# florianbaud/retrieval-augmented-mds

Hardware: AMD Instinct MI355X
Metric: MIPS queries/sec (exact top-5, bf16 index) (higher is better)
Workload: dtype bf16

## Files before the change

retrieval-augmented-mds_amd/csrc/scan_kernel_v4.hpp:

```cpp
#pragma once
#include <hip/hip_runtime.h>
#include <stdint.h>

#include "scan_kernel.hpp"
#include "scan_kernel_v3.hpp"

namespace mips {

typedef float f32x4 __attribute__((ext_vector_type(4)));

__device__ __forceinline__ unsigned lane_id_here() {
    unsigned ln = 0;
#if defined(__HIP_DEVICE_COMPILE__)
    asm volatile("v_mbcnt_lo_u32_b32 %0, -1, 0\n\tv_mbcnt_hi_u32_b32 %0, -1, %0" : "=v"(ln));
#endif
    return ln;
}

template <int KL, int KS32, int AD, int = 0, bool NT_DOCS = false, int PUB = 1>
__global__ __launch_bounds__(512, 2) void scan_kernel_v4(ScanArgs p) {
    extern __shared__ __attribute__((aligned(16))) unsigned char smem[];
    constexpr int WAVES = 8;
    constexpr int TN = WAVES * 32;
    constexpr int STAGES = 3;
    constexpr int STAGE_BYTES = V3_DB * KS32 * 64;
    constexpr int PIECES = STAGE_BYTES / 1024;
    constexpr int PPW = PIECES / WAVES;
    static_assert(PIECES % WAVES == 0, "every wave must issue the same number of DMA pieces");
    static_assert(KL <= 8, "8 class words vouch for 8 documents");
    static_assert(PUB >= 1 && PUB <= KL, "a sub-list publishes one of its entries");
    constexpr int STEPS = 2 * KS32;
    constexpr bool ONE_PASS = KL == 6 && KS32 == 24 && !NT_DOCS && PUB == 1;
    constexpr int KLI = ONE_PASS ? 4 : KL;
    static_assert(PUB <= KLI, "a sub-list publishes one of the entries it keeps");

    const int tid = threadIdx.x;
    const int lane = tid & 63;
    const int wave = __builtin_amdgcn_readfirstlane(tid >> 6);
    const int c = lane & 15;
    const int g = lane >> 4;

    const int xcd = blockIdx.x & 7;
    const int j = blockIdx.x >> 3;
    const int qt = (xcd % p.qgroups) + p.qgroups * (j % p.qt_per_group);
    const int split = (xcd / p.qgroups) * p.splits_per_group + j / p.qt_per_group;
    if (qt >= p.nqt) return;
    if (p.spin_limit < 0 && tid == 0) *p.err = 1u;
    const bool idle_wave = (qt * TN + wave * 32) >= p.nq;

    const int b0 = split * p.tiles_per_split;
    int b1 = b0 + p.tiles_per_split;
    if (b1 > p.ntiles) b1 = p.ntiles;
    const int nb = b1 > b0 ? b1 - b0 : 0;

    bf16x8 bq[2][KS32];
#pragma unroll
    for (int n = 0; n < 2; ++n) {
        const uint16_t* qrow = p.qbuf + ((int64_t)qt * TN + wave * 32 + n * 16 + c) * p.ld + 8 * g;
#pragma unroll
        for (int s = 0; s < KS32; ++s) bq[n][s] = *reinterpret_cast<const bf16x8*>(qrow + 32 * s);
#if defined(__HIP_DEVICE_COMPILE__)
#pragma unroll
        for (int s = 0; s < KS32; ++s) asm volatile("" : "+v"(bq[n][s]));
#endif
    }

    float ls[2][KLI];
    int li[2][KLI];
    float thr[2];
#pragma unroll
    for (int n = 0; n < 2; ++n) {
        thr[n] = -INFINITY;
#pragma unroll
        for (int i = 0; i < KLI; ++i) {
            ls[n][i] = -INFINITY;
            li[n][i] = IDX_NONE;
        }
    }

    constexpr unsigned THR_AREA = STAGES * STAGE_BYTES;
    constexpr unsigned THR_WAVE = 1024u;
    constexpr unsigned DUMP_AREA = THR_AREA + WAVES * THR_WAVE;
    static_assert(THR_AREA % 1024 == 0, "the wave areas are recovered from thr_addr by masking");
    auto thr_addr_of = [&](unsigned ln) { return THR_AREA + wave * THR_WAVE + ln * 16u; };
    *reinterpret_cast<uint4*>(smem + thr_addr_of(lane)) = make_uint4(0u, 0u, 0u, 0u);
    const __amdgpu_buffer_rsrc_t thr_rsrc = __builtin_amdgcn_make_buffer_rsrc(
        (void*)(reinterpret_cast<unsigned char*>(p.gthr) + (int64_t)qt * (WAVES * THR_WAVE) - (int64_t)THR_AREA), 0,
        (int)(THR_AREA + WAVES * THR_WAVE), 0x00020000);
    auto refresh_thresholds = [&](bool real) {
        lds_void* dst = (lds_void*)(smem + (real ? THR_AREA + wave * THR_WAVE : DUMP_AREA));
        const unsigned thr_addr = thr_addr_of(lane_id_here());
        __builtin_amdgcn_raw_ptr_buffer_load_lds(thr_rsrc, dst, 16, real ? thr_addr : (thr_addr | 0x40000000u), 0, 0, 16);
    };

    const unsigned char* docs_b = reinterpret_cast<const unsigned char*>(p.docs);
    const int64_t row_bytes = (int64_t)p.ld * 2;
    unsigned lane_off_kept = 0u;
    if constexpr (ONE_PASS) {
        lane_off_kept = ((unsigned)lane >> 3) * (unsigned)row_bytes + ((((unsigned)lane & 7u) ^ (((unsigned)lane >> 4) & 7u)) << 4);
#if defined(__HIP_DEVICE_COMPILE__)
        asm volatile("" : "+v"(lane_off_kept));
#endif
    }
    auto issue_piece = [&](const unsigned char* blk_base, int stage, int i) {
        const __amdgpu_buffer_rsrc_t rsrc =
            __builtin_amdgcn_make_buffer_rsrc((void*)blk_base, 0, (int)(V3_DB * row_bytes), 0x00020000);
        const int pc = wave + WAVES * i;
        const int slab = pc >> 2, rg = pc & 3;
        unsigned lane_off0 = lane_off_kept;
        if constexpr (!ONE_PASS) {
            const unsigned ln = __builtin_amdgcn_mbcnt_hi(~0u, __builtin_amdgcn_mbcnt_lo(~0u, 0u));
            lane_off0 = (ln >> 3) * (unsigned)row_bytes + (((ln & 7u) ^ ((ln >> 4) & 7u)) << 4);
        }
        __builtin_amdgcn_raw_ptr_buffer_load_lds(rsrc, (lds_void*)(smem + stage * STAGE_BYTES + pc * 1024), 16,
                                                 (rg & 1) ? (lane_off0 ^ 64u) : lane_off0,
                                                 rg * 8 * (int)row_bytes + slab * 128, 0, NT_DOCS ? 2 : 0);
    };
    auto issue = [&](const unsigned char* blk_base, int stage) {
#pragma unroll
        for (int i = 0; i < PPW; ++i) issue_piece(blk_base, stage, i);
    };

    auto rd0_of = [&](unsigned ln) {
        const unsigned cc = ln & 15u, gg = ln >> 4;
        return (int)(cc * 128u + ((gg ^ ((cc >> 1) & 7u)) << 4));
    };

    const unsigned cnt_lds = (unsigned)(size_t)(lds_void*)(smem + DUMP_AREA + 1024);
    unsigned arrivals_needed = 0;
    constexpr int PER_BLOCK = PPW + 1;
    auto arrive = [&]() {
        asm volatile("s_waitcnt vmcnt(%0)" ::"n"((STAGES - 2) * PER_BLOCK) : "memory");
#if defined(__HIP_DEVICE_COMPILE__)
        if (lane == 0) asm volatile("ds_add_u32 %0, %1" ::"v"(cnt_lds), "v"(1u) : "memory");
#endif
    };
    auto wait_all = [&]() {
        arrivals_needed += WAVES;
        for (int spin = 0;; ++spin) {
            unsigned v = 0;
#if defined(__HIP_DEVICE_COMPILE__)
            asm volatile("ds_read_b32 %0, %1\n\ts_waitcnt lgkmcnt(0)" : "=&v"(v) : "v"(cnt_lds) : "memory");
#endif
            if (__builtin_amdgcn_readfirstlane(v) >= arrivals_needed) break;
            if (spin > p.spin_limit) {
                if (lane == 0) *p.err = 1u;
                break;
            }
            __builtin_amdgcn_s_sleep(1);
        }
    };

    auto epilogue_half = [&](f32x4 (&acc)[2], int blk, int half) {
        const float mx0 = fmaxf(fmaxf(acc[0][0], acc[0][1]), fmaxf(acc[0][2], acc[0][3]));
        const float mx1 = fmaxf(fmaxf(acc[1][0], acc[1][1]), fmaxf(acc[1][2], acc[1][3]));
        if (__ballot(mx0 > thr[0] || mx1 > thr[1]) != 0ull) {
            const unsigned thr_addr = thr_addr_of(lane_id_here());
            const int base = blk * V3_DB + 16 * half + (int)((thr_addr >> 6) & 12u);
#pragma unroll
            for (int n = 0; n < 2; ++n) {
                const float mark = ls[n][PUB - 1];
#pragma unroll
                for (int r = 0; r < 4; ++r) {
                    const float s = acc[n][r];
                    if (s > thr[n]) {
                        list_insert<KLI>(ls[n], li[n], s, base + r);
                        thr[n] = fmaxf(thr[n], ls[n][KLI - 1]);
                    }
                }
                if (ls[n][PUB - 1] > mark) {
                    const unsigned cls = (4u * (unsigned)split + ((thr_addr >> 8) & 3u)) & 7u;
                    publish_umax(thr_encode(ls[n][PUB - 1]), (thr_addr & ~0x3FFu) + ((thr_addr & 0xF0u) << 1) + 512u * n + 4u * cls, thr_rsrc);
                }
            }
        }
    };

    auto epilogue_block = [&](f32x4 (&acc)[2][2], int blk) {
        const float mx0 = fmaxf(fmaxf(fmaxf(acc[0][0][0], acc[0][0][1]), fmaxf(acc[0][0][2], acc[0][0][3])),
                                fmaxf(fmaxf(acc[1][0][0], acc[1][0][1]), fmaxf(acc[1][0][2], acc[1][0][3])));
        const float mx1 = fmaxf(fmaxf(fmaxf(acc[0][1][0], acc[0][1][1]), fmaxf(acc[0][1][2], acc[0][1][3])),
                                fmaxf(fmaxf(acc[1][1][0], acc[1][1][1]), fmaxf(acc[1][1][2], acc[1][1][3])));
        if (__builtin_expect(__ballot((int)(mx0 > thr[0]) | (int)(mx1 > thr[1])) != 0ull, 0)) {
            const unsigned thr_addr = thr_addr_of(lane_id_here());
            const int base = blk * V3_DB + (int)((thr_addr >> 6) & 12u);
#pragma unroll
            for (int n = 0; n < 2; ++n) {
                const float mark = ls[n][PUB - 1];
                unsigned m = 0u;
#pragma unroll
                for (int e = 0; e < 8; ++e) m |= acc[e >> 2][n][e & 3] > thr[n] ? 1u << e : 0u;
                while (m != 0u) {
                    const int e = __ffs(m) - 1;
                    m &= m - 1u;
                    float s = acc[0][n][0];
#pragma unroll
                    for (int x = 1; x < 8; ++x) s = e == x ? acc[x >> 2][n][x & 3] : s;
                    if (s > thr[n]) {
                        list_insert<KLI>(ls[n], li[n], s, base + 16 * (e >> 2) + (e & 3));
                        thr[n] = fmaxf(thr[n], ls[n][KLI - 1]);
                    }
                }
                if (ls[n][PUB - 1] > mark) {
                    const unsigned cls = (4u * (unsigned)split + ((thr_addr >> 8) & 3u)) & 7u;
                    publish_umax(thr_encode(ls[n][PUB - 1]), (thr_addr & ~0x3FFu) + ((thr_addr & 0xF0u) << 1) + 512u * n + 4u * cls, thr_rsrc);
                }
            }
        }
    };

    auto block = [&](bool refresh, int blk, int stage, const unsigned char* pbase, int pstage) {
        if (idle_wave) {
            refresh_thresholds(false);
            issue(pbase, pstage);
            arrive();
            return;
        }
        const unsigned char* sa = smem + stage * STAGE_BYTES;
        const int rd0 = rd0_of(lane_id_here());
        auto lds_frag = [&](int t) {
            const int half = t / KS32, s = t % KS32;
            const int off = half * 2048 + (s >> 1) * 4096 + ((s & 1) ? (rd0 ^ 64) : rd0);
            return *reinterpret_cast<const bf16x8*>(sa + off);
        };
        bf16x8 ar[AD];
#pragma unroll
        for (int t = 0; t < AD; ++t) ar[t] = lds_frag(t);
        refresh_thresholds(refresh);
        __builtin_amdgcn_sched_barrier(0);
        const bool ragged = (int64_t)(blk + 1) * V3_DB > p.ntotal;
        auto mask_ragged = [&](f32x4 (&a)[2], int half) {
            const int base = blk * V3_DB + 16 * half + 4 * (int)(lane_id_here() >> 4);
#pragma unroll
            for (int r = 0; r < 4; ++r)
                if ((int64_t)(base + r) >= p.ntotal) {
                    a[0][r] = -INFINITY;
                    a[1][r] = -INFINITY;
                }
        };
        f32x4 accs[2][2];
#pragma unroll
        for (int half = 0; half < 2; ++half) {
            f32x4(&acc)[2] = accs[half];
#pragma unroll
            for (int n = 0; n < 2; ++n)
#pragma unroll
                for (int r = 0; r < 4; ++r) acc[n][r] = 0.f;
#pragma unroll
            for (int s = 0; s < KS32; ++s) {
                const int t = half * KS32 + s;
                acc[0] = __builtin_amdgcn_mfma_f32_16x16x32_bf16(ar[t % AD], bq[0][s], acc[0], 0, 0, 0);
                acc[1] = __builtin_amdgcn_mfma_f32_16x16x32_bf16(ar[t % AD], bq[1][s], acc[1], 0, 0, 0);
                if (t + AD < STEPS) ar[t % AD] = lds_frag(t + AD);
                if ((t % (STEPS / PPW)) == (STEPS / PPW) / 2) issue_piece(pbase, pstage, t / (STEPS / PPW));
                __builtin_amdgcn_sched_barrier(0);
            }
            if (half == 1) arrive();
            if (half == 1 && refresh) {
                const unsigned thr_addr = thr_addr_of(lane_id_here());
                const unsigned a0 = (unsigned)(size_t)(lds_void*)smem + (thr_addr & ~0x3FFu) + ((thr_addr & 0xF0u) << 1);
#pragma unroll
                for (int n = 0; n < 2; ++n) {
                    u32x4 w0 = {0u, 0u, 0u, 0u}, w1 = w0;
#if defined(__HIP_DEVICE_COMPILE__)
                    if (n == 0)
                        asm volatile("ds_read_b128 %0, %2\n\tds_read_b128 %1, %2 offset:16\n\ts_waitcnt lgkmcnt(0)"
                                     : "=&v"(w0), "=&v"(w1) : "v"(a0) : "memory");
                    else
                        asm volatile("ds_read_b128 %0, %2 offset:512\n\tds_read_b128 %1, %2 offset:528\n\ts_waitcnt lgkmcnt(0)"
                                     : "=&v"(w0), "=&v"(w1) : "v"(a0) : "memory");
#endif
                    const unsigned key = min(min(min(w0[0], w0[1]), min(w0[2], w0[3])), min(min(w1[0], w1[1]), min(w1[2], w1[3])));
                    thr[n] = fmaxf(thr[n], key > 1u ? thr_decode(key - 1u) : -INFINITY);
                }
            }
            if constexpr (!ONE_PASS) {
                if (ragged) mask_ragged(acc, half);
                epilogue_half(acc, blk, half);
            }
        }
        if constexpr (ONE_PASS) {
            if (ragged) {
                mask_ragged(accs[0], 0);
                mask_ragged(accs[1], 1);
            }
            epilogue_block(accs, blk);
        }
    };

    const unsigned char* first = docs_b + (int64_t)b0 * V3_DB * row_bytes;
    const unsigned char* last = docs_b + (int64_t)(b1 - 1) * V3_DB * row_bytes;
    const int64_t blk_bytes = V3_DB * row_bytes;
    constexpr int AHEAD = STAGES - 1;
    if (nb > 0) {
#pragma unroll
        for (int a = 0; a < AHEAD; ++a) {
            refresh_thresholds(true);
            issue(a < nb ? first + a * blk_bytes : last, a);
        }
    }
    const unsigned char* pbase = nb > AHEAD ? first + AHEAD * blk_bytes : last;
    int stage = 0, pstage = AHEAD;
    if (tid == 0) *reinterpret_cast<unsigned*>(smem + DUMP_AREA + 1024) = 0u;
    __syncthreads();
    if (nb > 0) arrive();
    for (int i = 0; i < nb; ++i) {
        wait_all();
        block(i < 8 || (i & 7) == 0, b0 + i, stage, pbase, pstage);
        if (i + AHEAD + 1 < nb) pbase += blk_bytes;
        stage = stage == STAGES - 1 ? 0 : stage + 1;
        pstage = pstage == STAGES - 1 ? 0 : pstage + 1;
    }
    asm volatile("s_waitcnt vmcnt(0)" ::: "memory");

#pragma unroll
    for (int n = 0; n < 2; ++n) {
        const int q = qt * TN + wave * 32 + n * 16 + c;
        const size_t o = (((size_t)q * p.nsplit + split) * 4 + g) * KL;
#pragma unroll
        for (int i = 0; i < KL; ++i) {
            p.part_s[o + i] = ls[n][i < KLI ? i : KLI - 1];
            p.part_i[o + i] = li[n][i < KLI ? i : KLI - 1];
        }
    }
}

}
```

Baseline: 907,700.

## Trim per-block scalar and address overhead in ONE_PASS scan kernel path

Result: faster. 936,000, median of 6 (+3.1%).

```diff
diff --git a/retrieval-augmented-mds_amd/csrc/scan_kernel_v4.hpp b/retrieval-augmented-mds_amd/csrc/scan_kernel_v4.hpp
--- a/retrieval-augmented-mds_amd/csrc/scan_kernel_v4.hpp
+++ b/retrieval-augmented-mds_amd/csrc/scan_kernel_v4.hpp
@@ -15,6 +15,16 @@
     asm volatile("v_mbcnt_lo_u32_b32 %0, -1, 0\n\tv_mbcnt_hi_u32_b32 %0, -1, %0" : "=v"(ln));
 #endif
     return ln;
+}
+
+__device__ __forceinline__ float max3_raw(float a, float b, float c) {
+    float r = a;
+#if defined(__HIP_DEVICE_COMPILE__)
+    asm volatile("v_max3_f32 %0, %1, %2, %3" : "=v"(r) : "v"(a), "v"(b), "v"(c));
+#else
+    (void)b; (void)c;
+#endif
+    return r;
 }
 
 template <int KL, int KS32, int AD, int = 0, bool NT_DOCS = false, int PUB = 1>
@@ -87,9 +97,16 @@
     const __amdgpu_buffer_rsrc_t thr_rsrc = __builtin_amdgcn_make_buffer_rsrc(
         (void*)(reinterpret_cast<unsigned char*>(p.gthr) + (int64_t)qt * (WAVES * THR_WAVE) - (int64_t)THR_AREA), 0,
         (int)(THR_AREA + WAVES * THR_WAVE), 0x00020000);
+    unsigned thr_addr_kept = 0u;
+    if constexpr (ONE_PASS) {
+        thr_addr_kept = thr_addr_of((unsigned)lane);
+#if defined(__HIP_DEVICE_COMPILE__)
+        asm volatile("" : "+v"(thr_addr_kept));
+#endif
+    }
     auto refresh_thresholds = [&](bool real) {
         lds_void* dst = (lds_void*)(smem + (real ? THR_AREA + wave * THR_WAVE : DUMP_AREA));
-        const unsigned thr_addr = thr_addr_of(lane_id_here());
+        const unsigned thr_addr = ONE_PASS ? thr_addr_kept : thr_addr_of(lane_id_here());
         __builtin_amdgcn_raw_ptr_buffer_load_lds(thr_rsrc, dst, 16, real ? thr_addr : (thr_addr | 0x40000000u), 0, 0, 16);
     };
 
@@ -125,12 +142,39 @@
         const unsigned cc = ln & 15u, gg = ln >> 4;
         return (int)(cc * 128u + ((gg ^ ((cc >> 1) & 7u)) << 4));
     };
+    unsigned rd0_kept = 0u, rd_even = 0u, rd_odd = 0u;
+    auto set_read_addresses = [&](int stage) {
+        const unsigned base = (unsigned)__builtin_amdgcn_readfirstlane((int)((unsigned)(size_t)(lds_void*)smem + (unsigned)(stage * STAGE_BYTES)));
+#if defined(__HIP_DEVICE_COMPILE__)
+        asm volatile("v_add_u32 %0, %3, %2\n\tv_xad_u32 %1, %2, 64, %3" : "=&v"(rd_even), "=v"(rd_odd) : "v"(rd0_kept), "s"(base));
+#else
+        (void)base;
+#endif
+    };
+    if constexpr (ONE_PASS) {
+        rd0_kept = (unsigned)rd0_of((unsigned)lane);
+#if defined(__HIP_DEVICE_COMPILE__)
+        asm volatile("" : "+v"(rd0_kept));
+#endif
+        set_read_addresses(0);
+    }
 
     const unsigned cnt_lds = (unsigned)(size_t)(lds_void*)(smem + DUMP_AREA + 1024);
     unsigned arrivals_needed = 0;
-    constexpr int PER_BLOCK = PPW + 1;
-    auto arrive = [&]() {
-        asm volatile("s_waitcnt vmcnt(%0)" ::"n"((STAGES - 2) * PER_BLOCK) : "memory");
+    static_assert(STAGES == 3, "arrive() lets the operations of one block stay in flight");
+    constexpr bool DUMMY_FETCH = !ONE_PASS;
+    auto arrive = [&](int fetched) {
+#if defined(__HIP_DEVICE_COMPILE__)
+        if constexpr (ONE_PASS) {
+            uint64_t exec_kept;
+            asm volatile("s_cmp_lg_u32 %3, 0\n\ts_cbranch_scc1 1f\n\ts_waitcnt vmcnt(%4)\n1:\n\ts_waitcnt vmcnt(%5)\n\t"
+                         "s_mov_b64 %0, exec\n\ts_mov_b64 exec, 1\n\tds_add_u32 %1, %2\n\ts_mov_b64 exec, %0"
+                         : "=&s"(exec_kept) : "v"(cnt_lds), "v"(1u), "s"(fetched), "n"(PPW), "n"(PPW + 1) : "memory", "scc");
+            return;
+        }
+#endif
+        if (fetched) asm volatile("s_waitcnt vmcnt(%0)" ::"n"(PPW + 1) : "memory");
+        else asm volatile("s_waitcnt vmcnt(%0)" ::"n"(PPW) : "memory");
 #if defined(__HIP_DEVICE_COMPILE__)
         if (lane == 0) asm volatile("ds_add_u32 %0, %1" ::"v"(cnt_lds), "v"(1u) : "memory");
 #endif
@@ -148,6 +192,26 @@
                 break;
             }
             __builtin_amdgcn_s_sleep(1);
+        }
+    };
+    auto reached = [&]() {
+        unsigned v = 0;
+#if defined(__HIP_DEVICE_COMPILE__)
+        asm volatile("ds_read_b32 %0, %1\n\ts_waitcnt lgkmcnt(0)" : "=&v"(v) : "v"(cnt_lds) : "memory");
+#endif
+        return __builtin_amdgcn_readfirstlane(v) >= arrivals_needed;
+    };
+    auto wait_all_straight = [&]() {
+        arrivals_needed += WAVES;
+        if (__builtin_expect(!reached(), 0)) {
+            for (int spin = 0;; ++spin) {
+                if (spin > p.spin_limit) {
+                    if (lane == 0) *p.err = 1u;
+                    break;
+                }
+                __builtin_amdgcn_s_sleep(1);
+                if (reached()) break;
+            }
         }
     };
 
@@ -176,11 +240,7 @@
         }
     };
 
-    auto epilogue_block = [&](f32x4 (&acc)[2][2], int blk) {
-        const float mx0 = fmaxf(fmaxf(fmaxf(acc[0][0][0], acc[0][0][1]), fmaxf(acc[0][0][2], acc[0][0][3])),
-                                fmaxf(fmaxf(acc[1][0][0], acc[1][0][1]), fmaxf(acc[1][0][2], acc[1][0][3])));
-        const float mx1 = fmaxf(fmaxf(fmaxf(acc[0][1][0], acc[0][1][1]), fmaxf(acc[0][1][2], acc[0][1][3])),
-                                fmaxf(fmaxf(acc[1][1][0], acc[1][1][1]), fmaxf(acc[1][1][2], acc[1][1][3])));
+    auto epilogue_block = [&](f32x4 (&acc)[2][2], int blk, float mx0, float mx1) {
         if (__builtin_expect(__ballot((int)(mx0 > thr[0]) | (int)(mx1 > thr[1])) != 0ull, 0)) {
             const unsigned thr_addr = thr_addr_of(lane_id_here());
             const int base = blk * V3_DB + (int)((thr_addr >> 6) & 12u);
@@ -209,26 +269,38 @@
         }
     };
 
-    auto block = [&](bool refresh, int blk, int stage, const unsigned char* pbase, int pstage) {
-        if (idle_wave) {
-            refresh_thresholds(false);
-            issue(pbase, pstage);
-            arrive();
-            return;
+    const int first_ragged = (int)(p.ntotal / V3_DB < 0x7fffffff ? p.ntotal / V3_DB : 0x7fffffff);
+    auto block = [&](int refresh_word, int blk, int stage, const unsigned char* pbase, int pstage) {
+        const bool refresh = refresh_word != 0;
+        if constexpr (!ONE_PASS) {
+            if (idle_wave) {
+                refresh_thresholds(false);
+                issue(pbase, pstage);
+                arrive(1);
+                return;
+            }
         }
         const unsigned char* sa = smem + stage * STAGE_BYTES;
-        const int rd0 = rd0_of(lane_id_here());
+        const int rd0 = ONE_PASS ? 0 : rd0_of(lane_id_here());
         auto lds_frag = [&](int t) {
             const int half = t / KS32, s = t % KS32;
+            if constexpr (ONE_PASS) {
+                typedef const __attribute__((address_space(3))) bf16x8 lds_frag_t;
+                return *(lds_frag_t*)(size_t)(((s & 1) ? rd_odd : rd_even) + (unsigned)(half * 2048 + (s >> 1) * 4096));
+            }
             const int off = half * 2048 + (s >> 1) * 4096 + ((s & 1) ? (rd0 ^ 64) : rd0);
             return *reinterpret_cast<const bf16x8*>(sa + off);
         };
         bf16x8 ar[AD];
 #pragma unroll
         for (int t = 0; t < AD; ++t) ar[t] = lds_frag(t);
-        refresh_thresholds(refresh);
+        if constexpr (DUMMY_FETCH) {
+            refresh_thresholds(refresh);
+        } else {
+            if (__builtin_expect(refresh, 0)) refresh_thresholds(true);
+        }
         __builtin_amdgcn_sched_barrier(0);
-        const bool ragged = (int64_t)(blk + 1) * V3_DB > p.ntotal;
+        const bool ragged = ONE_PASS ? blk >= first_ragged : (int64_t)(blk + 1) * V3_DB > p.ntotal;
         auto mask_ragged = [&](f32x4 (&a)[2], int half) {
             const int base = blk * V3_DB + 16 * half + 4 * (int)(lane_id_here() >> 4);
 #pragma unroll
@@ -239,6 +311,9 @@
                 }
         };
         f32x4 accs[2][2];
+        float mh[2] = {0.f, 0.f};
+        auto half_max = [&](const f32x4& a) { return max3_raw(max3_raw(a[0], a[1], a[2]), a[3], a[3]); };
+        auto block_max = [&](float m, const f32x4& a) { return max3_raw(max3_raw(m, a[0], a[1]), a[2], a[3]); };
 #pragma unroll
         for (int half = 0; half < 2; ++half) {
             f32x4(&acc)[2] = accs[half];
@@ -253,11 +328,19 @@
                 acc[1] = __builtin_amdgcn_mfma_f32_16x16x32_bf16(ar[t % AD], bq[1][s], acc[1], 0, 0, 0);
                 if (t + AD < STEPS) ar[t % AD] = lds_frag(t + AD);
                 if ((t % (STEPS / PPW)) == (STEPS / PPW) / 2) issue_piece(pbase, pstage, t / (STEPS / PPW));
+                if constexpr (ONE_PASS) {
+                    if (t == KS32 + 5) mh[0] = half_max(accs[0][0]);
+                    if (t == KS32 + 7) mh[1] = half_max(accs[0][1]);
+                    if (t == STEPS - AD) set_read_addresses(stage == STAGES - 1 ? 0 : stage + 1);
+                }
                 __builtin_amdgcn_sched_barrier(0);
             }
-            if (half == 1) arrive();
-            if (half == 1 && refresh) {
-                const unsigned thr_addr = thr_addr_of(lane_id_here());
+            if (half == 1) arrive(DUMMY_FETCH ? 1 : refresh_word);
+            if (half == 1 && (ONE_PASS ? __builtin_expect(refresh, 0) : refresh)) {
+                unsigned thr_addr = ONE_PASS ? thr_addr_kept : thr_addr_of(lane_id_here());
+#if defined(__HIP_DEVICE_COMPILE__)
+                if constexpr (ONE_PASS) asm volatile("" : "+v"(thr_addr));
+#endif
                 const unsigned a0 = (unsigned)(size_t)(lds_void*)smem + (thr_addr & ~0x3FFu) + ((thr_addr & 0xF0u) << 1);
 #pragma unroll
                 for (int n = 0; n < 2; ++n) {
@@ -280,11 +363,18 @@
             }
         }
         if constexpr (ONE_PASS) {
-            if (ragged) {
+            if (__builtin_expect(ragged, 0)) {
                 mask_ragged(accs[0], 0);
                 mask_ragged(accs[1], 1);
-            }
-            epilogue_block(accs, blk);
+                mh[0] = half_max(accs[0][0]);
+                mh[1] = half_max(accs[0][1]);
+            }
+#if defined(__HIP_DEVICE_COMPILE__)
+            asm volatile("s_nop 3" ::: "memory");
+#endif
+            const float mx0 = block_max(mh[0], accs[1][0]);
+            const float mx1 = block_max(mh[1], accs[1][1]);
+            epilogue_block(accs, blk, mx0, mx1);
         }
     };
 
@@ -303,13 +393,37 @@
     int stage = 0, pstage = AHEAD;
     if (tid == 0) *reinterpret_cast<unsigned*>(smem + DUMP_AREA + 1024) = 0u;
     __syncthreads();
-    if (nb > 0) arrive();
-    for (int i = 0; i < nb; ++i) {
-        wait_all();
-        block(i < 8 || (i & 7) == 0, b0 + i, stage, pbase, pstage);
+    if (nb > 0) arrive(1);
+    auto advance = [&](int i) {
         if (i + AHEAD + 1 < nb) pbase += blk_bytes;
         stage = stage == STAGES - 1 ? 0 : stage + 1;
         pstage = pstage == STAGES - 1 ? 0 : pstage + 1;
+    };
+    if constexpr (ONE_PASS) {
+        if (idle_wave) {
+            for (int i = 0; i < nb; ++i) {
+                wait_all_straight();
+                issue(pbase, pstage);
+                arrive(0);
+                advance(i);
+            }
+        } else {
+            for (int i = 0; i < nb; ++i) {
+                wait_all_straight();
+                int refresh_word = (int)(((unsigned)(i - 8) >> 31) | ((unsigned)((i & 7) - 1) >> 31));
+#if defined(__HIP_DEVICE_COMPILE__)
+                asm volatile("" : "+s"(refresh_word));
+#endif
+                block(refresh_word, b0 + i, stage, pbase, pstage);
+                advance(i);
+            }
+        }
+    } else {
+        for (int i = 0; i < nb; ++i) {
+            wait_all();
+            block(i < 8 || (i & 7) == 0 ? 1 : 0, b0 + i, stage, pbase, pstage);
+            advance(i);
+        }
     }
     asm volatile("s_waitcnt vmcnt(0)" ::: "memory");
 
```
